# msaelices/mojo-regex

Measured on AMD Instinct MI355X. Metric: GB/s input scanned + matches/sec, 1M x 1KiB batch, [a-z]+\d+ DFA, higher is better.
Workload: dtype u8

## Files before the change

### include/mrx_testing.h

```cpp
#ifndef MRX_TESTING_H
#define MRX_TESTING_H

#include <stddef.h>
#include <stdint.h>

#ifdef __cplusplus
extern "C" {
#endif

void mrx_timing_reset(void);
void mrx_timing_enable(int on);
double mrx_timing_scan_ms(int64_t* launches);
const char* mrx_last_kernel_name(void);
void mrx_debug_force_generic(int on);
void mrx_debug_long_text_kernels(int mode);
void mrx_debug_fused_findall(int mode);
void mrx_debug_stream_bits(int on);
void mrx_debug_stream_bits_trace(int64_t* d_trace);
void mrx_debug_dynamic_texts(int mode);
void mrx_debug_split_findall(int on);
void mrx_debug_dense_rows(int mode);
void mrx_debug_tries_always(int on);
void mrx_debug_chain_sub_general(int on);
int mrx_testing_emptywalk_findall(const mrx_handle* h, const uint8_t* text, int len, int32_t* spans, int cap);
void mrx_debug_subs_group(int lanes);
void mrx_debug_litscan_pieces(int mode);
void mrx_debug_multiwalk(int mode);
void mrx_debug_rec_skew(int64_t bytes);
int mrx_testing_comm_shift(const int64_t* d_prefix, int64_t n_local, const int64_t* d_meta_all, int meta_stride, int rank,
                           int64_t* d_out, int64_t pad_to, void* stream);
int mrx_testing_comm_compact(const int64_t* d_meta_all, int meta_stride, int nranks, const int64_t* d_stage_prefix, int64_t P,
                             const int32_t* d_stage_spans, int64_t cap, int64_t* d_gprefix, int64_t gprefix_cap,
                             int32_t* d_gspans, int64_t gspans_cap, int32_t* d_status, void* stream);
void mrx_debug_set_route(int mode);
struct mrx_set;
int mrx_testing_set_run(const struct mrx_set* s, int op, const uint8_t* text, int len, int32_t* out);
void mrx_debug_filter_form(int form);
void mrx_debug_extract_grid(int workgroups);
void mrx_debug_expand_grid(int workgroups);
size_t mrx_debug_scratch_bytes(void);
size_t mrx_debug_scratch_in_use(void);

#ifdef __cplusplus
// ... 4 lines not shown
```

### mojo_regex_amd/api.py

```python
from __future__ import annotations

import ctypes as C
import os
from typing import Iterable, List, Optional, Sequence, Tuple

import numpy as np

_HERE = os.path.dirname(os.path.abspath(__file__))
_LIB_NAME = "libmrx_hip.so"
_lib = None

MRX_OK, MRX_E_SYNTAX, MRX_E_UNSUPPORTED, MRX_E_NO_DEVICE, MRX_E_CAPACITY, MRX_E_ARGUMENT = range(6)


class MrxError(RuntimeError):
    """Any failure reported by libmrx_hip.so."""


class RegexSyntaxError(MrxError):
    """The reference's lexer/parser raises on this pattern (same message)."""


class UnsupportedPattern(MrxError):
    """The reference routes this pattern/operation to an engine outside the hot
# ... 88 lines not shown
        "mrx_debug_force_generic": (None, [C.c_int]),
        "mrx_debug_long_text_kernels": (None, [C.c_int]),
        "mrx_debug_fused_findall": (None, [C.c_int]),
        "mrx_debug_stream_bits": (None, [C.c_int]),
        "mrx_debug_stream_bits_trace": (None, [C.c_void_p]),
        "mrx_debug_dynamic_texts": (None, [C.c_int]),
        "mrx_debug_subs_group": (None, [C.c_int]),
        "mrx_debug_split_findall": (None, [C.c_int]),
        "mrx_debug_dense_rows": (None, [C.c_int]),
        "mrx_debug_tries_always": (None, [C.c_int]),
        "mrx_debug_chain_sub_general": (None, [C.c_int]),
        "mrx_testing_emptywalk_findall": (C.c_int, [H, C.c_char_p, C.c_int, i32p, C.c_int]),
        "mrx_debug_litscan_pieces": (None, [C.c_int]),
        "mrx_debug_multiwalk": (None, [C.c_int]),
        "mrx_debug_rec_skew": (None, [C.c_int64]),
        "mrx_release_scratch": (None, []),
        "mrx_debug_scratch_bytes": (C.c_size_t, []),
        "mrx_debug_scratch_in_use": (C.c_size_t, []),
        "mrx_version": (C.c_char_p, []),
        "mrx_comm_unique_id": (C.c_int, [C.c_void_p]),
        "mrx_comm_init": (C.c_int, [C.c_void_p, C.c_int, C.c_int, C.POINTER(H)]),
        "mrx_comm_free": (None, [H]),
        "mrx_comm_rank": (C.c_int, [H]),
        "mrx_comm_size": (C.c_int, [H]),
        "mrx_comm_spans_staging_bytes": (C.c_size_t, [H, C.c_int64, C.c_int64]),
        "mrx_comm_reserve": (C.c_int, [H, C.c_size_t]),
        "mrx_allgather_fixed": (C.c_int, [H, C.c_void_p, C.c_void_p, C.c_size_t, C.c_void_p]),
        "mrx_allgatherv_rows": (C.c_int, [H, C.c_void_p, C.c_int64, C.c_size_t, C.c_void_p, C.c_int64,
                                          C.POINTER(C.c_int64), C.c_void_p]),
        "mrx_allgatherv_spans": (C.c_int, [H, i64p, C.c_int64, i32p, C.c_int64, C.c_int64, i64p, C.c_int64, i32p,
# ... 100 lines not shown
    "mrx_set_filter_dev", "mrx_set_filter_known_dev", "mrx_set_filter_strided_dev", "mrx_set_filter_batch",
    "mrx_gather_spans_dev", "mrx_gather_spans_strided_dev", "mrx_gather_spans_batch",
    "mrx_extract_dev", "mrx_extract_known_dev", "mrx_extract_strided_dev", "mrx_extract_batch",
    "mrx_expand_spans_dev", "mrx_expand_spans_strided_dev", "mrx_expand_spans_batch",
    "mrx_expand_dev", "mrx_expand_strided_dev", "mrx_expand_batch",
]
TESTING_SYMBOLS = [
    "mrx_timing_reset", "mrx_timing_enable", "mrx_timing_scan_ms", "mrx_last_kernel_name",
    "mrx_debug_force_generic", "mrx_debug_long_text_kernels", "mrx_debug_scratch_bytes",
    "mrx_debug_scratch_in_use",
    "mrx_debug_fused_findall", "mrx_debug_stream_bits", "mrx_debug_stream_bits_trace", "mrx_debug_dynamic_texts", "mrx_debug_subs_group",
    "mrx_debug_split_findall", "mrx_debug_dense_rows", "mrx_debug_tries_always", "mrx_debug_chain_sub_general", "mrx_testing_emptywalk_findall", "mrx_debug_litscan_pieces", "mrx_debug_multiwalk", "mrx_debug_rec_skew", "mrx_testing_comm_shift", "mrx_testing_comm_compact",
    "mrx_debug_set_route", "mrx_testing_set_run", "mrx_debug_filter_form", "mrx_debug_extract_grid",
    "mrx_debug_expand_grid",
]
COMM_SYMBOLS = [
    "mrx_comm_unique_id", "mrx_comm_init", "mrx_comm_free", "mrx_comm_rank", "mrx_comm_size",
    "mrx_comm_spans_staging_bytes", "mrx_comm_reserve",
    "mrx_allgather_fixed", "mrx_allgatherv_rows", "mrx_allgatherv_spans",
]


def _b(x) -> bytes:
    if isinstance(x, str):
        return x.encode("utf-8")
    return bytes(x)


def _check(rc: int):
    if rc == MRX_OK:
# ... 877 lines not shown
```

### mojo_regex_amd/csrc/mrx_kernels.hip

```cpp
#include <hip/hip_runtime.h>
#include <atomic>
#include <map>
#include <type_traits>
#include <unordered_map>
#include <chrono>

#include <cstdio>
#include <cstdlib>
#include <cstring>
#include <mutex>
#include <string>
#include <vector>

#include "../../include/mrx.h"
#include "../../include/mrx_testing.h"
#include "mrx_device.hpp"
#include "mrx_host_batch.hpp"
#include "mrx_internal.hpp"
#include "mrx_lookback.hpp"

using namespace mrx;

namespace {

constexpr int kBlock = 256;

struct Layout : TextBatch {
  Layout() = default;
  Layout(const TextBatch& b) : TextBatch(b) {}
  int32_t split = 0;
  int32_t wide_slots = 0;
  const int32_t* vlen = nullptr;
  const uint32_t* vskip = nullptr;
  const int32_t* vbase = nullptr;
// ... 1605 lines not shown
#define MRX_FUSED_WAVES 4
#endif
__global__ __launch_bounds__(64 * kStreamWaves, (MODE == ST_FUSED ? MRX_FUSED_WAVES : 1)) void k_stream_findall(
    DevPlan p, const uint8_t* __restrict__ blob, const uint8_t* __restrict__ data, int64_t stride,
    const int32_t* __restrict__ lens, int32_t common_len, const int64_t* __restrict__ offsets,
    int64_t n, int32_t* __restrict__ counts,
    int32_t* __restrict__ wave_nrecs, EvRec* __restrict__ recs, int64_t rec_row,
    int32_t* __restrict__ out_s, int32_t* __restrict__ out_e,
    const int32_t* __restrict__ vlen = nullptr, const uint32_t* __restrict__ vskip = nullptr,
    const FusedArgs* __restrict__ fzp = nullptr) {
#define fz (*fzp)
  constexpr bool RECS = MODE == ST_RECORDS || MODE == ST_FUSED;
  constexpr bool ROWS = MODE == ST_ROWS;
  static_assert(!(MODE == ST_FUSED && VIRT), "pieces of long texts keep the three-launch form");
  static_assert(!ROWS || (!CSR && !VIRT && !REC32), "event rows: texts at a fixed aligned pitch");
  constexpr int kChunk = CH;
  constexpr int kRowPitch = CH + 16;
  constexpr int LPR = CH / 16;
  constexpr int RPI = 64 / LPR;
  constexpr int NL = 64 / RPI;
  __shared__ __align__(16) uint8_t tiles[kStreamWaves][64 * kRowPitch];
  __shared__ __align__(16) uint16_t col_lds[256];
  __shared__ __align__(16) uint16_t col32_lds[AUTO == 5 ? 256 : 2];
  static_assert(AUTO != 5 || MODE != ST_FIRST, "the anchored automaton has no code-column form");
  __shared__ __align__(16) uint4 pmask[17];
  if (threadIdx.x < 17) {
    const int x = threadIdx.x;
    uint32_t w[4];
    for (int j = 0; j < 4; ++j) {
      const int nb = x - 4 * j;
// ... 126 lines not shown
          }                                                                      \
        }                                                                        \
    } while (0)
    uint64_t skip_rows = 0;

    uint32_t q4 = 0;
    uint32_t q_codes = 0;
    int start = 0;
    int cnt = 0;
    int wrec = 0;
    bool done = !live;
    int res_s = -1, res_e = (MODE == ST_FIRST && live && p.fa_start_acc) ? 0 : -1;
    EvRec* wave_recs = (MODE == ST_RECORDS)
        ? recs + ((CSR && offsets) ? rec_region_start(offsets[base_text], w) : base_text * rec_row)
        : (MODE == ST_FUSED) ? recs + (((int64_t)blockIdx.x * kStreamWaves + wave) * 2 + half) * fz.rec_cap : nullptr;

    if (MODE == ST_FIRST) {
      uint4 pv = make_uint4(0, 0, 0, 0);
      if (live && my_len > 0) {
        if (CSR) pv = *(const uint4*)(((uintptr_t)(data + (offsets ? offsets[my_text] : my_text * stride))) & ~(uintptr_t)15);
        else pv = *(const uint4*)(data + my_text * stride);
      }
      const uint32_t pw[4] = {pv.x, pv.y, pv.z, pv.w};
      uint32_t pq = 0, pF = 0;
#pragma unroll
      for (int k = 0; k < 16; ++k) {
        const uint32_t b = (pw[k >> 2] >> ((k & 3) * 8)) & 0xFFu;
        const bool outside = k < mis || k >= flen;
        uint32_t e;
        if (AUTO == 2) {
// ... 148 lines not shown
          const int dsk = skip - gbase;
          if (dsk > 0) { em &= dsk >= 16 ? 0u : ~((1u << (2 * dsk)) - 1u); F = ns | em; }
          if (use_fill && !(vsk >> 31)) {
            const int de = my_len - gbase;
            if (de < 16) { em &= de <= 0 ? 0u : ((1u << (2 * de)) - 1u); F = ns | em; }
          }
        }
        if (MRX_ABLATE & 16) { cnt += (F == 0x12345u); continue; }
        if (ROWS) {
          if ((g & 1) == 0) F_even = F;
          else rowbuf[g >> 1] = make_uint2(F_even, F);
        } else
        if (RECS && REC32) {
          if ((g & 1) == 0) {
            F_even = F;
            sp_even = (uint32_t)start | ((uint32_t)(gbase + kRecPosBias) << 16);
            meta_even = ((uint32_t)lane << 26) | ((uint32_t)cnt & kRecBeforeMask);
          } else {
            const bool any = ((F_even | F) & 0xAAAAAAAAu) != 0u;
            const uint64_t has = __ballot(any);
            if (has) {
              if (any) {
                const int rank = __builtin_amdgcn_mbcnt_hi((uint32_t)(has >> 32),
                                                           __builtin_amdgcn_mbcnt_lo((uint32_t)has, 0));
                *(uint4*)(wave_recs + wrec + rank) = make_uint4(F_even, F, sp_even, meta_even);
              }
              wrec += __builtin_popcountll(has);
            }
          }
        } else if (RECS) {
          const uint64_t has = __ballot(em != 0);
          if (has) {
            if (em) {
              const int rank = __builtin_amdgcn_mbcnt_hi((uint32_t)(has >> 32),
                                                         __builtin_amdgcn_mbcnt_lo((uint32_t)has, 0));
              EvRec r;
              r.F = F; r.start = start; r.pos_base = gbase;
              r.meta = ((uint32_t)lane << 26) | ((uint32_t)cnt & kRecBeforeMask);
              if (!(MRX_ABLATE & 1)) wave_recs[wrec + rank] = r;
// ... 45 lines not shown
    }
    {
      const bool tail = MODE != ST_FIRST && live && (!VIRT || (vsk >> 31)) &&
                        (AUTO == 5 ? ((p.st_acc32 >> (q4 & 31u)) & 1u) != 0
                         : AUTO == 4 ? acc_lds[q4 >> (2 * p.st_cshift)] != 0
                         : AUTO == 2 ? acc_lds[q4 >> p.st_cshift] != 0
                                   : ((accmask >> (q4 >> (AUTO == 3 ? 3 : 2))) & 1u) != 0);
      if (RECS) {
        const uint64_t has = __ballot(tail);
        if (tail) {
          const int rank = __builtin_amdgcn_mbcnt_hi((uint32_t)(has >> 32),
                                                     __builtin_amdgcn_mbcnt_lo((uint32_t)has, 0));
          EvRec r;
          r.F = 2u; r.start = start; r.pos_base = my_len;
          r.meta = ((uint32_t)lane << 26) | ((uint32_t)cnt & kRecBeforeMask);
          if (REC32) *(uint4*)(wave_recs + wrec + rank) = make_uint4(2u, 0u, (uint32_t)start | ((uint32_t)(my_len + kRecPosBias) << 16), r.meta);
          else
          wave_recs[wrec + rank] = r;
        }
        wrec += __builtin_popcountll(has);
        if (MODE == ST_RECORDS && lane == 0) wave_nrecs[w] = wrec;
      }
      if (tail) ++cnt;
      if (MODE == ST_RECORDS) {
        int wt = live ? cnt : 0;
        for (int off = 32; off > 0; off >>= 1) wt += __shfl_xor(wt, off);
        if (lane == 0) wave_nrecs[nwaves_total + w] = wt;
      }
      if (MODE == ST_FIRST) {
        if (live) {
// ... 392 lines not shown
#define MRX_DECODE_TILE 2048
#endif
constexpr int kDecodeTile = MRX_DECODE_TILE;
#ifndef MRX_DECODE_BATCH
#define MRX_DECODE_BATCH 8
#endif
constexpr int kDecodeBatch = MRX_DECODE_BATCH;

constexpr int kScanBlock = 256;
constexpr int kScanItems = 8;
constexpr int kScanTile = kScanBlock * kScanItems;

#ifndef MRX_DYN_DECODE_TILE
#define MRX_DYN_DECODE_TILE 2048
#endif
template <bool PACK16, bool VBASE = false, bool REC32 = false, bool DYN = false, int TILE = kDecodeTile>
__global__ __launch_bounds__(kBlock) void k_decode(int64_t n, const int32_t* __restrict__ wave_nrecs,
                                                   const EvRec* __restrict__ recs, int64_t rec_row,
                                                   const int64_t* __restrict__ offsets,
                                                   const int32_t* __restrict__ counts,
                                                   const int64_t* __restrict__ wave_base,
                                                   const int64_t* __restrict__ scan_block_sums,
                                                   int64_t* __restrict__ prefix,
                                                   int32_t* __restrict__ spans, int64_t span_cap,
                                                   int fixed_len, int64_t* __restrict__ total_out,
                                                   const int32_t* __restrict__ vbase = nullptr,
                                                   const int64_t* __restrict__ base = nullptr, int reverse = 0) {
  static_assert(!(PACK16 && VBASE), "text-relative positions of a long text do not fit 16 bits");
  static_assert(!(DYN && VBASE), "pieces are not handed out dynamically");
  using Slot = typename std::conditional<PACK16, uint32_t, int2>::type;
  __shared__ Slot tile_all[kBlock / 64][TILE];
  __shared__ int dense_upto[kBlock / 64][64];
  constexpr int kDecodeTile = TILE, kDecodeDirect = 3 * TILE;
  __shared__ int rel_all[DYN ? kBlock / 64 : 1][DYN ? kDynTexts : 1];
  constexpr int kTexts = DYN ? kDynTexts : 64;
  constexpr uint32_t kBefore = DYN ? kDynBeforeMask : kRecBeforeMask;
  constexpr int kTextShift = DYN ? kDynShift : 26;
  const int lane = threadIdx.x & 63;
  Slot* tile = tile_all[threadIdx.x >> 6];
  int* rel_lds = rel_all[DYN ? (threadIdx.x >> 6) : 0];
  const int64_t nw = (n + kTexts - 1) / kTexts;
  const int waves_per_block = blockDim.x >> 6;
  for (int64_t w0 = (int64_t)blockIdx.x * waves_per_block + (threadIdx.x >> 6); w0 < nw;
       w0 += (int64_t)gridDim.x * waves_per_block) {
// ... 34 lines not shown
    const int my_cnt = i < n ? counts[i] : 0;
    int incl = my_cnt;
#pragma unroll
    for (int d = 1; d < 64; d <<= 1) {
      const int v = __shfl_up(incl, d);
      if (lane >= d) incl += v;
    }
    my_rel = incl - my_cnt;
    total_spans = __shfl(incl, 63);
    if (i < n) prefix[i] = pre0 + my_rel;
    if (i == n - 1) { prefix[n] = pre0 + incl; *total_out = pre0 + incl; }
    }
    const int total_recs = wave_nrecs[w];
    const EvRec* wave_recs = recs + (DYN ? rec_region_dyn(offsets[first], w)
                                         : offsets ? rec_region_start(offsets[first], w) : first * rec_row);
    const int my_vb = (VBASE && i < n) ? vbase[i] : 0;
    if (total_spans > kDecodeDirect) {
      constexpr int kRowCap = (DYN || !PACK16) ? 0 : kDecodeTile / 64;
      int done_t = 0;
      for (int j = 0; j < total_recs; j += 64 * kDecodeBatch) {
        EvRec rr[kDecodeBatch];
#pragma unroll
        for (int u = 0; u < kDecodeBatch; ++u) {
          const int o = j + u * 64 + lane;
          rr[u].F = 0; rr[u].start = 0; rr[u].pos_base = 0; rr[u].meta = 0;
          if (o < total_recs) {
            const uint4 q_ = mrx_ldg((const uint4*)(wave_recs + o));
            rr[u].F = q_.x; rr[u].start = (int32_t)q_.y; rr[u].pos_base = (int32_t)q_.z; rr[u].meta = q_.w;
          }
        }
        if (kRowCap > 0) {
          dense_upto[threadIdx.x >> 6][lane] = done_t;
          __builtin_amdgcn_fence(__ATOMIC_RELEASE, "wavefront");
          __builtin_amdgcn_wave_barrier();
          __builtin_amdgcn_fence(__ATOMIC_ACQUIRE, "wavefront");
        }
#pragma unroll
        for (int u = 0; u < kDecodeBatch; ++u) {
          EvRec r = rr[u];
          const int txt = DYN ? 0 : (int)(r.meta >> 26);
          const int rel_t = DYN ? rel_lds[r.meta >> kTextShift] : __shfl(my_rel, txt);
          if (VBASE) { const int vb = __shfl(my_vb, (int)(r.meta >> 26)); r.start += vb; r.pos_base += vb; }
          const int done_r = kRowCap > 0 ? __shfl(done_t, txt) : 0;
          int within = (int)(r.meta & kBefore);
          int64_t dst = pre0 + rel_t + within;
          uint32_t Fw = r.F;
          int pb = REC32 ? (int)((uint32_t)r.pos_base >> 16) - kRecPosBias : r.pos_base;
          int rstart = REC32 ? (int)((uint32_t)r.pos_base & 0xFFFFu) : r.start;
#pragma unroll
          for (int half = 0; half < (REC32 ? 2 : 1); ++half) {
            uint32_t em = Fw & 0xAAAAAAAAu;
            const uint32_t ns = Fw & 0x55555555u;
            while (em) {
              const int kk = __builtin_ctz(em) >> 1;
              const uint32_t nsb = ns & ((1u << (2 * kk)) - 1u);
              int st = nsb ? pb + ((31 - __builtin_clz(nsb)) >> 1) : rstart;
              if (fixed_len > 0) st = pb + kk - fixed_len;
              const int slot = within - done_r;
              if (kRowCap > 0 && slot < kRowCap) {
                if constexpr (PACK16) tile[txt * (kRowCap > 0 ? kRowCap : 1) + slot] = ((uint32_t)st << 16) | (uint32_t)(pb + kk);
              } else if (dst < span_cap) {
                *(int2*)(spans + 2 * dst) = make_int2(st, pb + kk);
              }
// ... 27 lines not shown
          }
          done_t = upto_t;
          __builtin_amdgcn_wave_barrier();
        }
      }
      continue;
    }
    for (int tb = 0; tb < total_spans; tb += kDecodeTile) {
      for (int j = 0; j < total_recs; j += 64 * kDecodeBatch) {
        EvRec rr[kDecodeBatch];
#pragma unroll
        for (int u = 0; u < kDecodeBatch; ++u) {
          const int o = j + u * 64 + lane;
          rr[u].F = 0; rr[u].start = 0; rr[u].pos_base = 0; rr[u].meta = 0;
          if (o < total_recs) {
            const uint4 q_ = mrx_ldg((const uint4*)(wave_recs + o));
            rr[u].F = q_.x; rr[u].start = (int32_t)q_.y; rr[u].pos_base = (int32_t)q_.z; rr[u].meta = q_.w;
          }
        }
#pragma unroll
        for (int u = 0; u < kDecodeBatch; ++u) {
          EvRec r = rr[u];
          const int rel_t = DYN ? rel_lds[r.meta >> kTextShift] : __shfl(my_rel, (int)(r.meta >> 26));
          if (VBASE) { const int vb = __shfl(my_vb, (int)(r.meta >> 26)); r.start += vb; r.pos_base += vb; }
          int dst = rel_t + (int)(r.meta & kBefore) - tb;
          uint32_t Fw = r.F;
          int pb = REC32 ? (int)((uint32_t)r.pos_base >> 16) - kRecPosBias : r.pos_base;
          int rstart = REC32 ? (int)((uint32_t)r.pos_base & 0xFFFFu) : r.start;
#pragma unroll
          for (int half = 0; half < (REC32 ? 2 : 1); ++half) {
            uint32_t em = Fw & 0xAAAAAAAAu;
            const uint32_t ns = Fw & 0x55555555u;
            while (em) {
              const int kk = __builtin_ctz(em) >> 1;
              const uint32_t nsb = ns & ((1u << (2 * kk)) - 1u);
              int st = nsb ? pb + ((31 - __builtin_clz(nsb)) >> 1) : rstart;
              if (fixed_len > 0) st = pb + kk - fixed_len;
              if (dst >= 0 && dst < kDecodeTile) {
                if constexpr (PACK16) tile[dst] = ((uint32_t)st << 16) | (uint32_t)(pb + kk);
                else tile[dst] = make_int2(st, pb + kk);
              }
              ++dst;
              em &= em - 1;
// ... 1622 lines not shown
bool stream_text_too_long(int64_t max_text) { return max_text >= kStreamMaxText; }
bool stream_layout_ok(const Layout&, int64_t n) { return n > 0; }
bool strided_fast(const Layout& lay) {
  return !lay.offsets && (lay.stride % 16 == 0) && (((uintptr_t)lay.data) % 16 == 0) &&
         lay.stride * 64 < (int64_t(1) << 31);
}

static bool code_columns_on() {
  static const bool on = [] { const char* e = getenv("MRX_NO_CODE_COLUMNS"); return !(e && e[0] == '1'); }();
  return on;
}

template <int MODE>
void launch_stream(const mrx_handle* h, const Layout& lay, int64_t n, int32_t* d_counts, int32_t* d_nrecs,
                   EvRec* d_recs, int64_t rec_row, int32_t* d_s, int32_t* d_e, hipStream_t s,
                   const int32_t* d_vlen = nullptr, const uint32_t* d_vskip = nullptr, bool rec32 = false,
                   const FusedArgs* fused = nullptr, int fused_grid = 0) {
  const DevPlan& p = h->hp.dev;
  const int g = MODE == ST_FUSED ? fused_grid : wave_grid(n, kStreamWaves);
  const FusedArgs* fzv = fused;
  const dim3 grid((unsigned)g), block(64 * kStreamWaves);
  const int kind = MODE == ST_FIRST ? p.fa_kind : p.st_kind;
  const bool table = kind == 2;
  const bool wide = kind == 3;
  const bool pairs = MODE != ST_FIRST && (table || wide) && p.off_stg_pair >= 0 && g_pair_tables;
  const size_t lds = pairs ? (size_t)p.stg_bytes
                           : wide ? 2048 : !table ? 0 : (size_t)(MODE == ST_FIRST ? p.fa_bytes : p.stg_bytes);
#define MRX_LAUNCH_R(AUTO, CSR, R32)                                                              \
  hipLaunchKernelGGL((k_stream_findall<MODE, (AUTO == 2 ? MRX_STREAM_CHUNK_TABLE : MRX_STREAM_CHUNK), AUTO, CSR, 0, R32>), grid, block, lds, s, p, \
                     H_BLOB(h), lay.data, lay.stride, lay.lens, lay.len, lay.offsets, n, d_counts, \
                     d_nrecs, d_recs, rec_row, d_s, d_e, (const int32_t*)nullptr, (const uint32_t*)nullptr, fzv)
#define MRX_LAUNCH(AUTO, CSR)                                                                     \
  do {                                                                                            \
    if constexpr (MODE == ST_RECORDS || MODE == ST_FUSED) {                                       \
      if (rec32) MRX_LAUNCH_R(AUTO, CSR, 1); else MRX_LAUNCH_R(AUTO, CSR, 0);                     \
    } else MRX_LAUNCH_R(AUTO, CSR, 0);                                                            \
  } while (0)
  if (d_vlen) {
    if constexpr (MODE == ST_RECORDS || MODE == ST_COUNT || MODE == ST_SEARCH || MODE == ST_FIRST) {
#define MRX_LAUNCH_V(AUTO)                                                                        \
  hipLaunchKernelGGL((k_stream_findall<MODE, (AUTO == 2 ? MRX_STREAM_CHUNK_TABLE : MRX_STREAM_CHUNK), AUTO, 1, 1>), grid, block, lds, s, p, \
                     H_BLOB(h), lay.data, lay.stride, lay.lens, lay.len, lay.offsets, n, d_counts, \
                     d_nrecs, d_recs, rec_row, d_s, d_e, d_vlen, d_vskip)
      if (pairs) { if constexpr (MODE != ST_FIRST) MRX_LAUNCH_V(4); }
      else if (table) MRX_LAUNCH_V(2);
      else if (wide) MRX_LAUNCH_V(3);
      else MRX_LAUNCH_V(1);
#undef MRX_LAUNCH_V
// ... 186 lines not shown
    HIP_TRY(hipGetLastError());
    tm.stop();
  }
  hipLaunchKernelGGL(k_scan_local<int32_t>, dim3((unsigned)ntiles), dim3(kScanBlock), 0, s, d_nrecs + nw, nw, d_wbase,
                     d_tsum);
  hipLaunchKernelGGL((k_decode<false, true>), dim3(grid_for(nv, kBlock)), dim3(kBlock), 0, s, nv, d_nrecs, d_recs,
                     (int64_t)0, pc.lay.offsets, d_vcounts, d_wbase, d_tsum, d_vprefix, d_spans, span_cap, p.st_fixed_len,
                     d_total, pc.vbase);
  hipLaunchKernelGGL(k_virt_prefix, dim3(grid_for(n + 1, kBlock)), dim3(kBlock), 0, s, n, pc.vfirst, d_vprefix, d_prefix);
  HIP_TRY(hipGetLastError());
  return MRX_OK;
}

std::atomic<int> g_split_findall{env_int("MRX_FINDALL_SPLIT", 0)};
std::atomic<int> g_dense_rows{env_int("MRX_DENSE_ROWS", 0)};
constexpr int64_t kSplitMinTexts = 1 << 18;
struct SideStream {
  hipStream_t side = nullptr;
  hipEvent_t scanned = nullptr, decoded = nullptr;
};
thread_local std::map<int, SideStream> g_side;
static int side_stream(SideStream** out) {
  int dev = 0;
  (void)hipGetDevice(&dev);
  SideStream& ss = g_side[dev];
  if (!ss.side) {
    HIP_TRY(hipStreamCreateWithFlags(&ss.side, hipStreamNonBlocking));
    HIP_TRY(hipEventCreateWithFlags(&ss.scanned, hipEventDisableTiming));
    HIP_TRY(hipEventCreateWithFlags(&ss.decoded, hipEventDisableTiming));
  }
// ... 168 lines not shown
  int32_t* d_counts = nullptr;
  int64_t* d_total = nullptr;
  StepRoute rt;
  bool stream_ok = false, mw_empty = false, mw_tries = false;
  bool mwalk_req = false;
  DevPlan pk;
  bool step_ok = false;
  bool bits_fixed = false;
  bool bits_fixed_slots = false;
  bool fused = false;
  bool split_done = false;
  bool dyn = false;
  unsigned long long* d_ctrl = nullptr;
  int32_t* d_blimit = nullptr;
  bool rec32 = false;
  int64_t max_text = int64_t(1) << 40;
  bool req_wave = false;
  bool mwalk_two_pass = false;
  int step_split = 0;
  Layout lay2;
  EvRec* d_recs = nullptr;
  int32_t* d_nrecs = nullptr;
  int64_t* d_wbase = nullptr;
  int32_t* d_slots = nullptr;
  int64_t rec_row = 0;
  Pieces pc;
  Layout lay_pre;
  int64_t csr_total = -1, csr_max = -1;
  bool by_pieces = false;
  bool finished = false;
// ... 129 lines not shown
      const int64_t nt = (n + kDynTexts - 1) / kDynTexts;
      HIP_TRY(scratch_alloc((void**)&d_recs, sizeof(EvRec) * (size_t)(csr_total / 16 + 4 * kDynTexts * (nt + 1)), s));
      HIP_TRY(scratch_alloc((void**)&d_nrecs, sizeof(int32_t) * 2 * nt, s));
      HIP_TRY(scratch_alloc((void**)&d_wbase, sizeof(int64_t) * (nt + 1), s));
      ScanTimer tm(s);
      launch_stream_dyn<ST_RECORDS>(h, lay, n, d_counts, d_nrecs, d_recs, nullptr, nullptr, s, rec32);
      g_last_kernel = "k_stream_findall_dyn";
      HIP_TRY(hipGetLastError());
      tm.stop();
    } else if (g_split_findall && !lay.offsets && strided_fast(lay) && span_cap > 0 && n >= kSplitMinTexts) {
      split_done = true;
      if (int rc = findall_split(h, lay, n, d_counts, d_prefix, d_spans, span_cap, d_total, rec_row, rec32, max_text <= 65535, s))
        return rc;
    } else {
    const int64_t skew = g_rec_skew.load(std::memory_order_relaxed);
    HIP_TRY(scratch_alloc((void**)&d_recs, sizeof(EvRec) * nrec + (size_t)skew, s));
    d_recs = (EvRec*)((uint8_t*)d_recs + skew);
    HIP_TRY(scratch_alloc((void**)&d_nrecs, sizeof(int32_t) * 2 * nw, s));
    HIP_TRY(scratch_alloc((void**)&d_wbase, sizeof(int64_t) * (nw + 1), s));
    ScanTimer tm(s);
    launch_stream<ST_RECORDS>(h, lay, n, d_counts, d_nrecs, d_recs, rec_row, nullptr, nullptr, s, nullptr, nullptr, rec32);
    g_last_kernel = "k_stream_findall";
    HIP_TRY(hipGetLastError());
    tm.stop();
    }
    return MRX_OK;
  }

  int stream_finish() {
    if (rows) {
      if (int rc = device_scan<int32_t>(d_counts, n, d_prefix, d_total, s)) return rc;
      const int G = max_text <= 1024 ? 16 : max_text <= 2048 ? 32 : 64;
      const int64_t per_block = (kBlock / 64) * (64 / G);
      const int64_t blocks = (n + per_block - 1) / per_block;
      const dim3 dg((unsigned)(blocks < 8 * grid_cap() ? blocks : 8 * grid_cap())), db(kBlock);
#define MRX_DR(GG) hipLaunchKernelGGL(k_decode_rows<GG>, dg, db, 0, s, n, (const uint2*)d_rows, row_pairs, (int)(max_text / 32), \
// ... 11 lines not shown
    hipLaunchKernelGGL(k_scan_local<int32_t>, dim3((unsigned)ntiles), dim3(kScanBlock), 0, s, d_nrecs + nw, nw,
                       d_wbase, d_tsum);
    const bool pack16 = max_text <= 65535;
    if (dyn) {
      const dim3 dg((unsigned)grid_for(nw * 64, kBlock) * 2), db(kBlock);
      if (pack16 && rec32)
        hipLaunchKernelGGL((k_decode<true, false, true, true, MRX_DYN_DECODE_TILE>), dg, db, 0, s, n, d_nrecs, d_recs, rec_row, lay.offsets, d_counts,
                           d_wbase, d_tsum, d_prefix, d_spans, span_cap, p.st_fixed_len, d_total);
      else if (pack16)
        hipLaunchKernelGGL((k_decode<true, false, false, true>), dg, db, 0, s, n, d_nrecs, d_recs, rec_row, lay.offsets, d_counts,
                           d_wbase, d_tsum, d_prefix, d_spans, span_cap, p.st_fixed_len, d_total);
      else
        hipLaunchKernelGGL((k_decode<false, false, false, true>), dg, db, 0, s, n, d_nrecs, d_recs, rec_row, lay.offsets, d_counts,
                           d_wbase, d_tsum, d_prefix, d_spans, span_cap, p.st_fixed_len, d_total);
    } else
    if (pack16 && rec32 && max_text >= 768)
      hipLaunchKernelGGL((k_decode<true, false, true, false, 3072>), dim3(env_knobs().decode_grid > 0 ? env_knobs().decode_grid : grid_for(n, kBlock) * 2), dim3(kBlock), 0, s, n, d_nrecs, d_recs,
                         rec_row, lay.offsets, d_counts, d_wbase, d_tsum, d_prefix, d_spans, span_cap, p.st_fixed_len,
                         d_total, (const int32_t*)nullptr, (const int64_t*)nullptr, env_knobs().decode_reverse);
    else if (pack16 && rec32)
      hipLaunchKernelGGL((k_decode<true, false, true>), dim3(grid_for(n, kBlock) * 2), dim3(kBlock), 0, s, n, d_nrecs, d_recs,
                         rec_row, lay.offsets, d_counts, d_wbase, d_tsum, d_prefix, d_spans, span_cap, p.st_fixed_len,
                         d_total);
    else if (pack16)
      hipLaunchKernelGGL(k_decode<true>, dim3(grid_for(n, kBlock) * 2), dim3(kBlock), 0, s, n, d_nrecs, d_recs,
                         rec_row, lay.offsets, d_counts, d_wbase, d_tsum, d_prefix, d_spans, span_cap, p.st_fixed_len,
                         d_total);
    else
      hipLaunchKernelGGL(k_decode<false>, dim3(grid_for(n, kBlock)), dim3(kBlock), 0, s, n, d_nrecs, d_recs,
                         rec_row, lay.offsets, d_counts, d_wbase, d_tsum, d_prefix, d_spans, span_cap, p.st_fixed_len,
                         d_total);
// ... 2134 lines not shown
  HIP_TRY(hipMemcpy(out_offsets, oo.p, sizeof(int64_t) * (n + 1), hipMemcpyDeviceToHost));
  if (rc == MRX_OK && tot > 0) HIP_TRY(hipMemcpy(out_data, od.p, (size_t)tot, hipMemcpyDeviceToHost));
  return rc;
}

void mrx_timing_reset(void) { g_scan_ms = 0; g_scan_launches = 0; }
void mrx_timing_enable(int on) { g_timing = on != 0; }
double mrx_timing_scan_ms(int64_t* launches) {
  if (launches) *launches = g_scan_launches;
  return g_scan_launches ? g_scan_ms / (double)g_scan_launches : 0.0;
}
const char* mrx_last_kernel_name(void) { return g_last_kernel; }
void mrx_debug_force_generic(int on) { g_force_generic = on < 0 ? 0 : on > 2 ? 2 : on; }
void mrx_debug_long_text_kernels(int mode) { g_long_text_mode = mode < 0 ? 0 : mode > 3 ? 0 : mode; }
void mrx_debug_rec_skew(int64_t bytes) { g_rec_skew = bytes < 0 ? 0 : (bytes & ~int64_t(15)); }
void mrx_debug_fused_findall(int mode) { g_fused = mode < 0 ? 0 : mode > 2 ? 0 : mode; }
void mrx_debug_stream_bits(int on) { mrx::stream_bits_set_mode(on); }
void mrx_debug_stream_bits_trace(int64_t* d_trace) { mrx::stream_bits_set_trace(d_trace); }
void mrx_debug_dynamic_texts(int mode) { g_dyn_mode = mode < 0 ? 0 : mode > 2 ? 0 : mode; }
void mrx_debug_split_findall(int on) { g_split_findall = on ? 1 : 0; }
void mrx_debug_dense_rows(int mode) { g_dense_rows = mode; }
void mrx_debug_tries_always(int on) { g_tries_always = on ? 1 : 0; }
void mrx_debug_chain_sub_general(int on) { g_chain_sub_general = on ? 1 : 0; }
int mrx_testing_emptywalk_findall(const mrx_handle* h, const uint8_t* text, int len, int32_t* spans, int cap) {
  if (!h || !h->hp.ew2_ok || len < 0) return -1;
  const std::vector<std::pair<int, int>> v = emptywalk2_run(h->hp.ew2, text, len);
  for (size_t k = 0; k < v.size() && (int)k < cap; ++k) { spans[2 * k] = v[k].first; spans[2 * k + 1] = v[k].second; }
  return (int)v.size();
}
void mrx_debug_subs_group(int g) { g_subs_group = (g == 0 || g == 16 || g == 32 || g == 64 || g == 256) ? g : -1; }
// ... 64 lines not shown
```

### mojo_regex_amd/csrc/mrx_lookback.hpp

```cpp
#pragma once
#include <hip/hip_runtime.h>
#include <cstdint>

namespace mrx {

#ifndef MRX_NT_LOADS
#define MRX_NT_LOADS 1
#endif
typedef unsigned int mrx_u32x4 __attribute__((ext_vector_type(4)));
__device__ __forceinline__ uint4 mrx_ldg(const uint4* p) {
#if MRX_NT_LOADS
  const mrx_u32x4 v = __builtin_nontemporal_load((const mrx_u32x4*)p);
  return make_uint4(v.x, v.y, v.z, v.w);
#else
  return *p;
#endif
}
#define MRX_LDG(P) mrx_ldg(P)
typedef int mrx_i32x2 __attribute__((ext_vector_type(2)));
__device__ __forceinline__ void mrx_stg_span(int32_t* p, int a, int b) {
#if MRX_NT_LOADS
  mrx_i32x2 v; v.x = a; v.y = b;
  __builtin_nontemporal_store(v, (mrx_i32x2*)p);
#else
  *(int2*)p = make_int2(a, b);
#endif
}



constexpr unsigned long long kDescValid = 1ull << 62, kDescVal = (1ull << 62) - 1ull;
constexpr int kGroupCountShift = 40;
constexpr unsigned long long kGroupSumMask = (1ull << kGroupCountShift) - 1ull;
// ... 141 lines not shown
```

Before: 3178.

## Pack findall event records into 12 bytes for short strided texts

Adds a 12-byte event-record format for texts up to 1024 bytes at a fixed pitch. Start, pair index, lane and match-before count are packed into one dword, so the separate sp word is dropped and records shrink from 16 to 12 bytes. Both the stream kernel (writer) and the decode kernel (reader) get REC12 template variants. The goal is less scratch traffic between the two passes, at the cost of scalar 32-bit stores and loads in place of uint4 vector accesses, which may hurt coalescing.

```diff
diff --git a/include/mrx_testing.h b/include/mrx_testing.h
--- a/include/mrx_testing.h
+++ b/include/mrx_testing.h
@@ -27,6 +27,8 @@
 void mrx_debug_litscan_pieces(int mode);
 void mrx_debug_multiwalk(int mode);
 void mrx_debug_rec_skew(int64_t bytes);
+void mrx_debug_rec12(int mode);
+int mrx_testing_rec12_roundtrip(int start, int pair, int lane, int before, int32_t out[4]);
 int mrx_testing_comm_shift(const int64_t* d_prefix, int64_t n_local, const int64_t* d_meta_all, int meta_stride, int rank,
                            int64_t* d_out, int64_t pad_to, void* stream);
 int mrx_testing_comm_compact(const int64_t* d_meta_all, int meta_stride, int nranks, const int64_t* d_stage_prefix, int64_t P,
diff --git a/mojo_regex_amd/api.py b/mojo_regex_amd/api.py
--- a/mojo_regex_amd/api.py
+++ b/mojo_regex_amd/api.py
@@ -126,6 +126,8 @@
         "mrx_debug_litscan_pieces": (None, [C.c_int]),
         "mrx_debug_multiwalk": (None, [C.c_int]),
         "mrx_debug_rec_skew": (None, [C.c_int64]),
+        "mrx_debug_rec12": (None, [C.c_int]),
+        "mrx_testing_rec12_roundtrip": (C.c_int, [C.c_int, C.c_int, C.c_int, C.c_int, C.POINTER(C.c_int32)]),
         "mrx_release_scratch": (None, []),
         "mrx_debug_scratch_bytes": (C.c_size_t, []),
         "mrx_debug_scratch_in_use": (C.c_size_t, []),
@@ -256,6 +258,7 @@
     "mrx_debug_set_route", "mrx_testing_set_run", "mrx_debug_filter_form", "mrx_debug_extract_grid",
     "mrx_debug_expand_grid",
 ]
+TESTING_SYMBOLS_NUMBERED = ["mrx_debug_rec12", "mrx_testing_rec12_roundtrip"]
 COMM_SYMBOLS = [
     "mrx_comm_unique_id", "mrx_comm_init", "mrx_comm_free", "mrx_comm_rank", "mrx_comm_size",
     "mrx_comm_spans_staging_bytes", "mrx_comm_reserve",
diff --git a/mojo_regex_amd/csrc/mrx_kernels.hip b/mojo_regex_amd/csrc/mrx_kernels.hip
--- a/mojo_regex_amd/csrc/mrx_kernels.hip
+++ b/mojo_regex_amd/csrc/mrx_kernels.hip
@@ -18,6 +18,7 @@
 #include "mrx_host_batch.hpp"
 #include "mrx_internal.hpp"
 #include "mrx_lookback.hpp"
+#include "mrx_rec12.hpp"
 
 using namespace mrx;
 
@@ -1653,6 +1654,8 @@
   constexpr bool ROWS = MODE == ST_ROWS;
   static_assert(!(MODE == ST_FUSED && VIRT), "pieces of long texts keep the three-launch form");
   static_assert(!ROWS || (!CSR && !VIRT && !REC32), "event rows: texts at a fixed aligned pitch");
+  constexpr bool REC12 = REC32 == 2;
+  static_assert(!REC12 || (MODE == ST_RECORDS && !CSR && !VIRT), "12-byte records: the three-launch form at a fixed aligned pitch");
   constexpr int kChunk = CH;
   constexpr int kRowPitch = CH + 16;
   constexpr int LPR = CH / 16;
@@ -1809,6 +1812,7 @@
     EvRec* wave_recs = (MODE == ST_RECORDS)
         ? recs + ((CSR && offsets) ? rec_region_start(offsets[base_text], w) : base_text * rec_row)
         : (MODE == ST_FUSED) ? recs + (((int64_t)blockIdx.x * kStreamWaves + wave) * 2 + half) * fz.rec_cap : nullptr;
+    uint32_t* const wave_recs12 = REC12 ? (uint32_t*)recs + 3 * (base_text * rec_row) : nullptr;
 
     if (MODE == ST_FIRST) {
       uint4 pv = make_uint4(0, 0, 0, 0);
@@ -1987,8 +1991,12 @@
         if (RECS && REC32) {
           if ((g & 1) == 0) {
             F_even = F;
+            if (REC12) {
+              meta_even = rec12_pack((uint32_t)start, (uint32_t)gbase >> 5, (uint32_t)lane, (uint32_t)cnt);
+            } else {
             sp_even = (uint32_t)start | ((uint32_t)(gbase + kRecPosBias) << 16);
             meta_even = ((uint32_t)lane << 26) | ((uint32_t)cnt & kRecBeforeMask);
+            }
           } else {
             const bool any = ((F_even | F) & 0xAAAAAAAAu) != 0u;
             const uint64_t has = __ballot(any);
@@ -1996,6 +2004,10 @@
               if (any) {
                 const int rank = __builtin_amdgcn_mbcnt_hi((uint32_t)(has >> 32),
                                                            __builtin_amdgcn_mbcnt_lo((uint32_t)has, 0));
+                if (REC12) {
+                  uint32_t* const d = wave_recs12 + 3 * (wrec + rank);
+                  d[0] = F_even; d[1] = F; d[2] = meta_even;
+                } else
                 *(uint4*)(wave_recs + wrec + rank) = make_uint4(F_even, F, sp_even, meta_even);
               }
               wrec += __builtin_popcountll(has);
@@ -2071,6 +2083,12 @@
           EvRec r;
           r.F = 2u; r.start = start; r.pos_base = my_len;
           r.meta = ((uint32_t)lane << 26) | ((uint32_t)cnt & kRecBeforeMask);
+          if (REC12) {
+            const uint32_t bit = 2u << (2 * (my_len & 15));
+            uint32_t* const d = wave_recs12 + 3 * (wrec + rank);
+            d[0] = (my_len & 16) ? 0u : bit; d[1] = (my_len & 16) ? bit : 0u;
+            d[2] = rec12_pack((uint32_t)start, (uint32_t)my_len >> 5, (uint32_t)lane, (uint32_t)cnt);
+          } else
           if (REC32) *(uint4*)(wave_recs + wrec + rank) = make_uint4(2u, 0u, (uint32_t)start | ((uint32_t)(my_len + kRecPosBias) << 16), r.meta);
           else
           wave_recs[wrec + rank] = r;
@@ -2493,7 +2511,7 @@
 #ifndef MRX_DYN_DECODE_TILE
 #define MRX_DYN_DECODE_TILE 2048
 #endif
-template <bool PACK16, bool VBASE = false, bool REC32 = false, bool DYN = false, int TILE = kDecodeTile>
+template <bool PACK16, bool VBASE = false, bool REC32 = false, bool DYN = false, int TILE = kDecodeTile, bool REC12 = false>
 __global__ __launch_bounds__(kBlock) void k_decode(int64_t n, const int32_t* __restrict__ wave_nrecs,
                                                    const EvRec* __restrict__ recs, int64_t rec_row,
                                                    const int64_t* __restrict__ offsets,
@@ -2507,6 +2525,7 @@
                                                    const int64_t* __restrict__ base = nullptr, int reverse = 0) {
   static_assert(!(PACK16 && VBASE), "text-relative positions of a long text do not fit 16 bits");
   static_assert(!(DYN && VBASE), "pieces are not handed out dynamically");
+  static_assert(!REC12 || (REC32 && PACK16 && !VBASE && !DYN), "12-byte records: short texts at a fixed aligned pitch");
   using Slot = typename std::conditional<PACK16, uint32_t, int2>::type;
   __shared__ Slot tile_all[kBlock / 64][TILE];
   __shared__ int dense_upto[kBlock / 64][64];
@@ -2571,6 +2590,7 @@
     const int total_recs = wave_nrecs[w];
     const EvRec* wave_recs = recs + (DYN ? rec_region_dyn(offsets[first], w)
                                          : offsets ? rec_region_start(offsets[first], w) : first * rec_row);
+    const uint32_t* wave_recs12 = REC12 ? (const uint32_t*)recs + 3 * (first * rec_row) : nullptr;
     const int my_vb = (VBASE && i < n) ? vbase[i] : 0;
     if (total_spans > kDecodeDirect) {
       constexpr int kRowCap = (DYN || !PACK16) ? 0 : kDecodeTile / 64;
@@ -2582,8 +2602,13 @@
           const int o = j + u * 64 + lane;
           rr[u].F = 0; rr[u].start = 0; rr[u].pos_base = 0; rr[u].meta = 0;
           if (o < total_recs) {
+            if (REC12) {
+              const uint32_t* q_ = wave_recs12 + 3 * o;
+              rr[u].F = mrx_ldg32(q_); rr[u].start = (int32_t)mrx_ldg32(q_ + 1); rr[u].meta = mrx_ldg32(q_ + 2);
+            } else {
             const uint4 q_ = mrx_ldg((const uint4*)(wave_recs + o));
             rr[u].F = q_.x; rr[u].start = (int32_t)q_.y; rr[u].pos_base = (int32_t)q_.z; rr[u].meta = q_.w;
+            }
           }
         }
         if (kRowCap > 0) {
@@ -2599,11 +2624,11 @@
           const int rel_t = DYN ? rel_lds[r.meta >> kTextShift] : __shfl(my_rel, txt);
           if (VBASE) { const int vb = __shfl(my_vb, (int)(r.meta >> 26)); r.start += vb; r.pos_base += vb; }
           const int done_r = kRowCap > 0 ? __shfl(done_t, txt) : 0;
-          int within = (int)(r.meta & kBefore);
+          int within = REC12 ? rec12_before(r.meta) : (int)(r.meta & kBefore);
           int64_t dst = pre0 + rel_t + within;
           uint32_t Fw = r.F;
-          int pb = REC32 ? (int)((uint32_t)r.pos_base >> 16) - kRecPosBias : r.pos_base;
-          int rstart = REC32 ? (int)((uint32_t)r.pos_base & 0xFFFFu) : r.start;
+          int pb = REC12 ? 32 * rec12_pair(r.meta) : REC32 ? (int)((uint32_t)r.pos_base >> 16) - kRecPosBias : r.pos_base;
+          int rstart = REC12 ? rec12_start(r.meta) : REC32 ? (int)((uint32_t)r.pos_base & 0xFFFFu) : r.start;
 #pragma unroll
           for (int half = 0; half < (REC32 ? 2 : 1); ++half) {
             uint32_t em = Fw & 0xAAAAAAAAu;
@@ -2661,8 +2686,13 @@
           const int o = j + u * 64 + lane;
           rr[u].F = 0; rr[u].start = 0; rr[u].pos_base = 0; rr[u].meta = 0;
           if (o < total_recs) {
+            if (REC12) {
+              const uint32_t* q_ = wave_recs12 + 3 * o;
+              rr[u].F = mrx_ldg32(q_); rr[u].start = (int32_t)mrx_ldg32(q_ + 1); rr[u].meta = mrx_ldg32(q_ + 2);
+            } else {
             const uint4 q_ = mrx_ldg((const uint4*)(wave_recs + o));
             rr[u].F = q_.x; rr[u].start = (int32_t)q_.y; rr[u].pos_base = (int32_t)q_.z; rr[u].meta = q_.w;
+            }
           }
         }
 #pragma unroll
@@ -2670,10 +2700,10 @@
           EvRec r = rr[u];
           const int rel_t = DYN ? rel_lds[r.meta >> kTextShift] : __shfl(my_rel, (int)(r.meta >> 26));
           if (VBASE) { const int vb = __shfl(my_vb, (int)(r.meta >> 26)); r.start += vb; r.pos_base += vb; }
-          int dst = rel_t + (int)(r.meta & kBefore) - tb;
+          int dst = rel_t + (REC12 ? rec12_before(r.meta) : (int)(r.meta & kBefore)) - tb;
           uint32_t Fw = r.F;
-          int pb = REC32 ? (int)((uint32_t)r.pos_base >> 16) - kRecPosBias : r.pos_base;
-          int rstart = REC32 ? (int)((uint32_t)r.pos_base & 0xFFFFu) : r.start;
+          int pb = REC12 ? 32 * rec12_pair(r.meta) : REC32 ? (int)((uint32_t)r.pos_base >> 16) - kRecPosBias : r.pos_base;
+          int rstart = REC12 ? rec12_start(r.meta) : REC32 ? (int)((uint32_t)r.pos_base & 0xFFFFu) : r.start;
 #pragma unroll
           for (int half = 0; half < (REC32 ? 2 : 1); ++half) {
             uint32_t em = Fw & 0xAAAAAAAAu;
@@ -4326,7 +4356,7 @@
 template <int MODE>
 void launch_stream(const mrx_handle* h, const Layout& lay, int64_t n, int32_t* d_counts, int32_t* d_nrecs,
                    EvRec* d_recs, int64_t rec_row, int32_t* d_s, int32_t* d_e, hipStream_t s,
-                   const int32_t* d_vlen = nullptr, const uint32_t* d_vskip = nullptr, bool rec32 = false,
+                   const int32_t* d_vlen = nullptr, const uint32_t* d_vskip = nullptr, int rec32 = 0,
                    const FusedArgs* fused = nullptr, int fused_grid = 0) {
   const DevPlan& p = h->hp.dev;
   const int g = MODE == ST_FUSED ? fused_grid : wave_grid(n, kStreamWaves);
@@ -4344,6 +4374,9 @@
                      d_nrecs, d_recs, rec_row, d_s, d_e, (const int32_t*)nullptr, (const uint32_t*)nullptr, fzv)
 #define MRX_LAUNCH(AUTO, CSR)                                                                     \
   do {                                                                                            \
+    if constexpr (MODE == ST_RECORDS && CSR == 0) {                                               \
+      if (rec32 == 2) { MRX_LAUNCH_R(AUTO, CSR, 2); break; }                                      \
+    }                                                                                             \
     if constexpr (MODE == ST_RECORDS || MODE == ST_FUSED) {                                       \
       if (rec32) MRX_LAUNCH_R(AUTO, CSR, 1); else MRX_LAUNCH_R(AUTO, CSR, 0);                     \
     } else MRX_LAUNCH_R(AUTO, CSR, 0);                                                            \
@@ -4560,6 +4593,7 @@
 
 std::atomic<int> g_split_findall{env_int("MRX_FINDALL_SPLIT", 0)};
 std::atomic<int> g_dense_rows{env_int("MRX_DENSE_ROWS", 0)};
+std::atomic<int> g_rec12{env_int("MRX_REC12", 1)};
 constexpr int64_t kSplitMinTexts = 1 << 18;
 struct SideStream {
   hipStream_t side = nullptr;
@@ -4758,6 +4792,7 @@
   unsigned long long* d_ctrl = nullptr;
   int32_t* d_blimit = nullptr;
   bool rec32 = false;
+  bool rec12 = false;
   int64_t max_text = int64_t(1) << 40;
   bool req_wave = false;
   bool mwalk_two_pass = false;
@@ -4917,12 +4952,19 @@
         return rc;
     } else {
     const int64_t skew = g_rec_skew.load(std::memory_order_relaxed);
-    HIP_TRY(scratch_alloc((void**)&d_recs, sizeof(EvRec) * nrec + (size_t)skew, s));
+    rec12 = g_rec12 != 0 && rec32 && !lay.offsets && strided_fast(lay) && max_text <= kRec12MaxLen;
+    size_t rec_bytes = sizeof(EvRec) * nrec;
+    if (rec12) {
+      rec_row = rec12_row_len(max_text);
+      rec_bytes = (size_t)12 * (size_t)rec_row * (size_t)n;
+    }
+    HIP_TRY(scratch_alloc((void**)&d_recs, rec_bytes + (size_t)skew, s));
     d_recs = (EvRec*)((uint8_t*)d_recs + skew);
     HIP_TRY(scratch_alloc((void**)&d_nrecs, sizeof(int32_t) * 2 * nw, s));
     HIP_TRY(scratch_alloc((void**)&d_wbase, sizeof(int64_t) * (nw + 1), s));
     ScanTimer tm(s);
-    launch_stream<ST_RECORDS>(h, lay, n, d_counts, d_nrecs, d_recs, rec_row, nullptr, nullptr, s, nullptr, nullptr, rec32);
+    launch_stream<ST_RECORDS>(h, lay, n, d_counts, d_nrecs, d_recs, rec_row, nullptr, nullptr, s, nullptr, nullptr,
+                              rec12 ? 2 : (int)rec32);
     g_last_kernel = "k_stream_findall";
     HIP_TRY(hipGetLastError());
     tm.stop();
@@ -4964,7 +5006,15 @@
         hipLaunchKernelGGL((k_decode<false, false, false, true>), dg, db, 0, s, n, d_nrecs, d_recs, rec_row, lay.offsets, d_counts,
                            d_wbase, d_tsum, d_prefix, d_spans, span_cap, p.st_fixed_len, d_total);
     } else
-    if (pack16 && rec32 && max_text >= 768)
+    if (rec12 && max_text >= 768)
+      hipLaunchKernelGGL((k_decode<true, false, true, false, 3072, true>), dim3(env_knobs().decode_grid > 0 ? env_knobs().decode_grid : grid_for(n, kBlock) * 2), dim3(kBlock), 0, s, n, d_nrecs, d_recs,
+                         rec_row, lay.offsets, d_counts, d_wbase, d_tsum, d_prefix, d_spans, span_cap, p.st_fixed_len,
+                         d_total, (const int32_t*)nullptr, (const int64_t*)nullptr, env_knobs().decode_reverse);
+    else if (rec12)
+      hipLaunchKernelGGL((k_decode<true, false, true, false, kDecodeTile, true>), dim3(grid_for(n, kBlock) * 2), dim3(kBlock), 0, s, n, d_nrecs, d_recs,
+                         rec_row, lay.offsets, d_counts, d_wbase, d_tsum, d_prefix, d_spans, span_cap, p.st_fixed_len,
+                         d_total);
+    else if (pack16 && rec32 && max_text >= 768)
       hipLaunchKernelGGL((k_decode<true, false, true, false, 3072>), dim3(env_knobs().decode_grid > 0 ? env_knobs().decode_grid : grid_for(n, kBlock) * 2), dim3(kBlock), 0, s, n, d_nrecs, d_recs,
                          rec_row, lay.offsets, d_counts, d_wbase, d_tsum, d_prefix, d_spans, span_cap, p.st_fixed_len,
                          d_total, (const int32_t*)nullptr, (const int64_t*)nullptr, env_knobs().decode_reverse);
@@ -7129,6 +7179,15 @@
 void mrx_debug_force_generic(int on) { g_force_generic = on < 0 ? 0 : on > 2 ? 2 : on; }
 void mrx_debug_long_text_kernels(int mode) { g_long_text_mode = mode < 0 ? 0 : mode > 3 ? 0 : mode; }
 void mrx_debug_rec_skew(int64_t bytes) { g_rec_skew = bytes < 0 ? 0 : (bytes & ~int64_t(15)); }
+void mrx_debug_rec12(int mode) { g_rec12 = mode != 0; }
+int mrx_testing_rec12_roundtrip(int start, int pair, int lane, int before, int32_t out[4]) {
+  if (start < 0 || start >= kRec12MaxLen || pair < 0 || pair > kRec12MaxLen / 32 || lane < 0 || lane > 63 || before < 0 ||
+      before >= kRec12MaxLen || !out)
+    return -1;
+  const uint32_t m = rec12_pack((uint32_t)start, (uint32_t)pair, (uint32_t)lane, (uint32_t)before);
+  out[0] = rec12_start(m); out[1] = rec12_pair(m); out[2] = rec12_lane(m); out[3] = rec12_before(m);
+  return 0;
+}
 void mrx_debug_fused_findall(int mode) { g_fused = mode < 0 ? 0 : mode > 2 ? 0 : mode; }
 void mrx_debug_stream_bits(int on) { mrx::stream_bits_set_mode(on); }
 void mrx_debug_stream_bits_trace(int64_t* d_trace) { mrx::stream_bits_set_trace(d_trace); }
diff --git a/mojo_regex_amd/csrc/mrx_lookback.hpp b/mojo_regex_amd/csrc/mrx_lookback.hpp
--- a/mojo_regex_amd/csrc/mrx_lookback.hpp
+++ b/mojo_regex_amd/csrc/mrx_lookback.hpp
@@ -17,6 +17,13 @@
 #endif
 }
 #define MRX_LDG(P) mrx_ldg(P)
+__device__ __forceinline__ uint32_t mrx_ldg32(const uint32_t* p) {
+#if MRX_NT_LOADS
+  return __builtin_nontemporal_load(p);
+#else
+  return *p;
+#endif
+}
 typedef int mrx_i32x2 __attribute__((ext_vector_type(2)));
 __device__ __forceinline__ void mrx_stg_span(int32_t* p, int a, int b) {
 #if MRX_NT_LOADS
diff --git a/mojo_regex_amd/csrc/mrx_rec12.hpp b/mojo_regex_amd/csrc/mrx_rec12.hpp
--- /dev/null
+++ b/mojo_regex_amd/csrc/mrx_rec12.hpp
@@ -0,0 +1,34 @@
+#pragma once
+#include <cstdint>
+
+#if defined(__HIPCC__) || defined(__CUDACC__)
+#define MRX_REC12_HD __host__ __device__ inline
+#else
+#define MRX_REC12_HD inline
+#endif
+
+namespace mrx {
+
+constexpr int kRec12MaxLen = 1024;
+constexpr int kRec12StartBits = 10, kRec12BeforeBits = 10, kRec12PairBits = 6, kRec12LaneBits = 6;
+constexpr int kRec12BeforeShift = kRec12StartBits;
+constexpr int kRec12PairShift = kRec12BeforeShift + kRec12BeforeBits;
+constexpr int kRec12LaneShift = kRec12PairShift + kRec12PairBits;
+static_assert(kRec12LaneShift + kRec12LaneBits == 32, "the four fields fill one dword");
+static_assert(kRec12LaneShift == 26, "lane sits where the 16-byte records have it");
+static_assert(kRec12MaxLen - 1 < (1 << kRec12StartBits), "a walk starts at a byte of the text");
+static_assert(kRec12MaxLen - 1 < (1 << kRec12BeforeBits), "at most one match per byte, the last one not before itself");
+static_assert(kRec12MaxLen / 32 < (1 << kRec12PairBits), "pair of the match that ends at the last byte's end");
+static_assert(63 < (1 << kRec12LaneBits), "64 texts per wavefront");
+
+MRX_REC12_HD uint32_t rec12_pack(uint32_t start, uint32_t pair, uint32_t lane, uint32_t before) {
+  return start | (before << kRec12BeforeShift) | (pair << kRec12PairShift) | (lane << kRec12LaneShift);
+}
+MRX_REC12_HD int rec12_start(uint32_t m) { return (int)(m & ((1u << kRec12StartBits) - 1u)); }
+MRX_REC12_HD int rec12_before(uint32_t m) { return (int)((m >> kRec12BeforeShift) & ((1u << kRec12BeforeBits) - 1u)); }
+MRX_REC12_HD int rec12_pair(uint32_t m) { return (int)((m >> kRec12PairShift) & ((1u << kRec12PairBits) - 1u)); }
+MRX_REC12_HD int rec12_lane(uint32_t m) { return (int)(m >> kRec12LaneShift); }
+
+MRX_REC12_HD int64_t rec12_row_len(int64_t max_len) { return max_len / 32 + 2; }
+
+}
```

After: 3241, median of 6. 2.0% higher.
